# holstegelab/otter

Measured on AMD Instinct MI355X. Metric: regions/sec (otter assemble) on synthetic TR BED+BAM, 1/2/4/8 MI355X, higher is better.
Workload: dtype i16

## Files before the change

otter_amd/csrc/wfa_affine.hip:

```cpp
#include "wfa_affine_common.hpp"
#include "wfa_affine_reg.hpp"
#include "otg_chain.hpp"
#include "otg_match_queue.hpp"
#include <algorithm>
#include <cstdlib>
#include <mutex>
#include <vector>

using namespace otg_affine;

namespace {

template <int WPB>
__global__ __launch_bounds__(WPB * 64) void wfa_affine_kernel(
    const uint8_t* __restrict__ arena, const otg_align_task* __restrict__ tasks,
    const uint32_t* __restrict__ todo, const uint32_t* __restrict__ n_todo_ptr, uint32_t n_todo_imm,
    int xs, int oes, int es, int g,
    int32_t* __restrict__ scores, const uint64_t* __restrict__ cig_off, uint32_t* __restrict__ cig_len,
    uint8_t* __restrict__ cig_arena, uint64_t* __restrict__ cells,
    uint32_t* __restrict__ ticket, uint32_t* __restrict__ n_overflow, uint32_t* __restrict__ overflow_list,
    AffWs ws)
{
  constexpr int QCAP = 2048;
  __shared__ int s_lo[WPB][3][64];
// ... 734 lines not shown
  uint32_t* todo = (uint32_t*)otg_slot(ctx, SLOT_TODO, 4 * (size_t)n_tasks * sizeof(uint32_t));
  if (!cnt || !todo) return OTG_ERR_HIP;

  const size_t maxlen = ((size_t)ctx->max_seq_len + 4095) & ~(size_t)4095;
  AffWs ws = aff_ws_common(maxlen, xs, oes, es);
  ws.dbg = otg_env_set("OTG_DEBUG") ? 1 : 0; ws.visited = &cnt->visited;
  aff_ws_layout(ws, true);

  static const bool no_v3 = otg_env_set("OTG_NO_AFFINE_V3");
  static const bool no_bound = otg_env_set("OTG_NO_AFFINE_BOUND");
  static const int reg_mask_env = otg_env_int("OTG_AFFINE_REG", 31);
  static const int shape_env = otg_env_int("OTG_REG_SHAPE", 0);
  const int shape[OTG_REG_TIERS] = {(shape_env / 10000) % 10, (shape_env / 1000) % 10, (shape_env / 100) % 10, (shape_env / 10) % 10, shape_env % 10};
  const bool bounded = !no_v3 && es == 1 && xs == 2 && oes == 4 && !no_bound;
  int reg_mask = !bounded ? 0 : (maxlen <= 4096 ? (reg_mask_env & ~16) : reg_mask_env) & 31;

  constexpr int NWA = 4;
  constexpr int WPB = 4;
  AffWs wsA = ws, wsB = ws, wsC = ws, wr[OTG_REG_TIERS];
  uint32_t wavesA = 0, wavesB = 0, gridC = 2, blocks[OTG_REG_TIERS] = {0, 0, 0, 0, 0};
  const uint32_t ncu = (uint32_t)ctx->n_cu;
  {
    std::lock_guard<std::mutex> alloc_lock(otg_device_mutex(ctx->device));
    size_t free_b = 0, total_b = 0;
    HIP_TRY(ctx, hipMemGetInfo(&free_b, &total_b));
    const size_t budget = std::min<size_t>((size_t)(total_b * 0.2), (size_t)((free_b + ctx->pool[SLOT_WF_WS].cap) * 0.8));
    auto fit = [&](uint32_t& nwaves, size_t& slab) {
      while (nwaves > 1 && (ws.off_slab + slab) * (size_t)nwaves > budget) {
        if (slab > ((size_t)4 << 20)) slab /= 2; else nwaves = (nwaves + 1) / 2;
      }
    };
    auto diamond_slab = [&](size_t window) { return std::min<size_t>((size_t)(0.2 * (double)maxlen * (double)maxlen), window * window * 5 / 8) + (1 << 16); };
    wavesA = ncu * 2; size_t slabA = diamond_slab(4096);
    fit(wavesA, slabA);
    aff_ws_slab(wsA, slabA);
    wavesB = maxlen > 8192 ? ncu : ncu / 2; size_t slabB = diamond_slab(12288);
    fit(wavesB, slabB);
    aff_ws_slab(wsB, slabB);
    size_t slabC = std::min<size_t>((size_t)2 * maxlen * (size_t)(ws.nrows), budget / (gridC * WPB));
    static const size_t slab_cap_env = (size_t)otg_env_int("OTG_AFFINE_LAST_SLAB_MB", 0) << 20;
    if (slab_cap_env) slabC = std::min(slabC, slab_cap_env);
    if (slabC > ws.off_slab + 256) slabC -= ws.off_slab + 256;
    aff_ws_slab(wsC, slabC);
    const size_t need = std::max(std::max(wsA.stride * wavesA, wsB.stride * wavesB), wsC.stride * (size_t)gridC * WPB);
    uint8_t* wsp = (uint8_t*)otg_slot(ctx, SLOT_WF_WS, need);
    if (!wsp) return OTG_ERR_HIP;
    wsA.base = wsB.base = wsC.base = wsp;

    if (reg_mask) {
      HIP_TRY(ctx, hipMemGetInfo(&free_b, &total_b));
      const size_t budget_r = std::min<size_t>((size_t)(total_b * 0.25), (size_t)((free_b + ctx->pool[SLOT_REVOPS].cap) * 0.8));
      uint32_t al[OTG_REG_TIERS];
      for (int t = 0; t < OTG_REG_TIERS; ++t) {
        AffWs w = ws;
        const size_t cap = (size_t)OTG_REG_CAP[t];
        w.nrows = OTG_REG_CAP[t] + 64;
        aff_ws_layout(w, false);
        size_t slab = cap * cap * 7 / 8 + (1 << 16);
        if (t == 4) slab = std::min<size_t>(slab, (size_t)(0.2 * (double)maxlen * (double)maxlen) + (1 << 20));
        aff_ws_slab(w, slab);
        wr[t] = w;
        int apb = 1, bpc = 1;
        otg_affine_reg_geometry(t, shape[t], &apb, &bpc);
        blocks[t] = (reg_mask >> t) & 1 ? ncu * (uint32_t)bpc : 0u;
        al[t] = blocks[t] * (uint32_t)apb;
      }
      auto total = [&]() { size_t s = 256; for (int t = 0; t < OTG_REG_TIERS; ++t) s += wr[t].stride * al[t]; return s; };
      while (total() > budget_r) {
        int t = -1;
        if (blocks[4] > ncu / 4 && (wr[4].stride * al[4] >= wr[3].stride * al[3] || blocks[3] <= ncu / 2)) t = 4;
        else if (blocks[3] > ncu / 2) t = 3;
        if (t >= 0) { blocks[t] /= 2; al[t] = blocks[t]; continue; }
        for (t = OTG_REG_TIERS - 1; t >= 0 && !blocks[t]; --t) {}
        if (t < 0) break;
        blocks[t] = 0; al[t] = 0; reg_mask &= ~(1 << t);
      }
      uint8_t* wsr = reg_mask ? (uint8_t*)otg_slot(ctx, SLOT_REVOPS, total()) : nullptr;
      if (reg_mask && !wsr) {
        (void)hipGetLastError();
        reg_mask = 0;
      }
      if (ws.dbg) fprintf(stderr, "[otg] affine: register tiers keep %u / %u / %u / %u / %u alignments in flight, workspaces %.1f GB of a budget of %.1f GB, mask %d\n",
                          al[0], al[1], al[2], al[3], al[4], (double)total() / 1e9, (double)budget_r / 1e9, reg_mask);
      uint8_t* p = wsr;
      for (int t = 0; t < OTG_REG_TIERS; ++t) { wr[t].base = p; if (p) p += wr[t].stride * al[t]; }
    }
  }

  uint32_t* listA = todo;
  uint32_t* listB = todo + n_tasks;
  uint32_t* sorted = todo + 2 * (size_t)n_tasks;
  uint32_t* ovf_r = todo + 3 * (size_t)n_tasks;
  if (kernel_ms) HIP_TRY(ctx, hipEventRecord(ctx->ev0, ctx->stream));
  OtgTodo cur{d_todo, d_n_todo, n_tasks};
  if (!no_v3 && es == 1) {
    int32_t* d_bound = nullptr;
    if (bounded) {
      d_bound = (int32_t*)otg_slot(ctx, SLOT_BT_POOL, (size_t)n_tasks * sizeof(int32_t));
      if (!d_bound) return OTG_ERR_HIP;
      auto launch_bound = [&](auto kernel, uint32_t wpb, uint32_t bpc) {
        const uint32_t gridU = std::min<uint32_t>(ncu * bpc, (n_tasks + wpb - 1) / wpb);
        hipLaunchKernelGGL(kernel, dim3(gridU), dim3(wpb * 64), 0, ctx->stream, d_arena, d_tasks, d_todo, d_n_todo, n_tasks, d_bound, &cnt->bound_ticket);
      };
      if (maxlen <= 8192) launch_bound(wfa_affine_bound1_kernel<2, 4, 1030, 4>, 4, 8);
      else if (maxlen <= 12288) launch_bound(wfa_affine_bound1_kernel<2, 4, 1542, 4>, 4, 6);
      else if (maxlen <= 16384) launch_bound(wfa_affine_bound1_kernel<2, 4, 2054, 4>, 4, 4);
      else launch_bound(wfa_affine_bound1_kernel<2, 4, 4102, 2>, 2, 4);
    }
    if (d_bound && reg_mask) {
      uint32_t* hist = (uint32_t*)otg_slot(ctx, SLOT_ROWTAB, TSORT_BUCKETS * sizeof(uint32_t));
      uint32_t* seg = cnt->seg; uint32_t* n_ovf = &cnt->reg_overflow;
      if (!hist) return OTG_ERR_HIP;
      HIP_TRY(ctx, hipMemsetAsync(hist, 0, TSORT_BUCKETS * sizeof(uint32_t), ctx->stream));
      const uint32_t sg = std::min<uint32_t>((n_tasks + 2047) / 2048, ncu * 2);
      hipLaunchKernelGGL(K_tsort_hist, dim3(sg), dim3(256), 0, ctx->stream, d_todo, d_n_todo, n_tasks, d_tasks, (const int32_t*)d_bound, hist, reg_mask);
      hipLaunchKernelGGL(K_tsort_scan, dim3(1), dim3(1024), 0, ctx->stream, hist, seg);
      hipLaunchKernelGGL(K_tsort_scatter, dim3(sg), dim3(256), 0, ctx->stream, d_todo, d_n_todo, n_tasks, d_tasks, (const int32_t*)d_bound, hist, sorted, reg_mask);
      hipLaunchKernelGGL(K_seg_copy, dim3(std::min<uint32_t>((n_tasks + 255) / 256, 1024u)), dim3(256), 0, ctx->stream, (const uint32_t*)sorted,
                         (const uint32_t*)(seg + OTG_REG_TIERS), ovf_r, n_ovf);
      static const int conc_env = otg_env_int("OTG_AFFINE_CONCURRENT", -1);
      const bool concurrent = conc_env >= 0 ? conc_env != 0 : n_tasks <= 50000u;
      hipStream_t main_stream = ctx->stream;
      if (concurrent) {
        if (!ctx->ev_fork) {
          HIP_TRY(ctx, hipEventCreateWithFlags(&ctx->ev_fork, hipEventDisableTiming));
          for (int t = 0; t < OTG_REG_TIERS; ++t) {
            HIP_TRY(ctx, hipStreamCreateWithFlags(&ctx->tier_stream[t], hipStreamNonBlocking));
            HIP_TRY(ctx, hipEventCreateWithFlags(&ctx->ev_join[t], hipEventDisableTiming));
          }
        }
        HIP_TRY(ctx, hipEventRecord(ctx->ev_fork, main_stream));
      }
      int side_of[OTG_REG_TIERS] = {-2, -2, -2, -2, -2};
      int order[OTG_REG_TIERS] = {4, 3, 2, 1, 0};
      if (concurrent) {
        uint32_t hseg[OTG_REG_TIERS + 2];
        HIP_TRY(ctx, hipMemcpyAsync(hseg, seg, sizeof(hseg), hipMemcpyDeviceToHost, main_stream));
        HIP_TRY(ctx, hipStreamSynchronize(main_stream));
        static const double weight[OTG_REG_TIERS] = {1.0, 2.2, 4.0, 16.0, 64.0};
        double cost[OTG_REG_TIERS], load[3] = {0.0, 0.0, 0.0};
        for (int t = 0; t < OTG_REG_TIERS; ++t) cost[t] = blocks[t] ? weight[t] * (double)(hseg[t + 1] - hseg[t]) : 0.0;
        std::sort(order, order + OTG_REG_TIERS, [&](int a, int b) { return cost[a] > cost[b]; });
        for (int q = 0; q < OTG_REG_TIERS; ++q) {
          const int t = order[q];
          if (cost[t] <= 0.0) continue;
          int best = 0;
          for (int j = 1; j < 3; ++j) if (load[j] < load[best]) best = j;
          load[best] += cost[t];
          side_of[t] = best - 1;
        }
      } else {
        for (int t = 0; t < OTG_REG_TIERS; ++t) side_of[t] = blocks[t] ? -1 : -2;
      }
      bool side_used[2] = {false, false};
      int rc = OTG_OK; hipError_t he = hipSuccess;
      for (int q = 0; q < OTG_REG_TIERS && !rc; ++q) {
        const int t = order[q], sd = side_of[t];
        if (sd == -2) continue;
        if (sd >= 0 && !side_used[sd] && (he = hipStreamWaitEvent(ctx->tier_stream[sd], ctx->ev_fork, 0)) != hipSuccess) break;
        if (sd >= 0) { side_used[sd] = true; ctx->stream = ctx->tier_stream[sd]; }
        rc = otg_launch_affine_reg_tier(ctx, t, shape[t], blocks[t], d_arena, d_tasks, sorted, seg + t, g, d_scores, d_cig_off, d_cig_len, d_cig_arena, d_cells,
                                        &cnt->reg_ticket[t], n_ovf, ovf_r, wr[t], d_bound, &cnt->visited);
        ctx->stream = main_stream;
      }
      for (int sd = 0; sd < 2; ++sd) if (side_used[sd]) {
        if (!rc && he == hipSuccess && (he = hipEventRecord(ctx->ev_join[sd], ctx->tier_stream[sd])) == hipSuccess) he = hipStreamWaitEvent(main_stream, ctx->ev_join[sd], 0);
// ... 132 lines not shown
```

otter_amd/csrc/wfa_affine_reg.hip:

```cpp
#include "wfa_affine_common.hpp"
#include "wfa_affine_reg.hpp"
#include <cstdlib>

using namespace otg_affine;

namespace {

typedef short otg_short2 __attribute__((ext_vector_type(2)));
typedef unsigned short otg_ushort2 __attribute__((ext_vector_type(2)));

template <int I, int N, class F> __device__ __forceinline__ void static_for(F&& f)
{
  if constexpr (I < N) { f(std::integral_constant<int, I>{}); static_for<I + 1, N>(f); }
}
__device__ __forceinline__ otg_short2 as_s2(uint32_t a) { otg_short2 x; __builtin_memcpy(&x, &a, 4); return x; }
__device__ __forceinline__ otg_ushort2 as_u2(uint32_t a) { otg_ushort2 x; __builtin_memcpy(&x, &a, 4); return x; }
__device__ __forceinline__ uint32_t from_s2(otg_short2 x) { uint32_t o; __builtin_memcpy(&o, &x, 4); return o; }
__device__ __forceinline__ uint32_t from_u2(otg_ushort2 x) { uint32_t o; __builtin_memcpy(&o, &x, 4); return o; }
__device__ __forceinline__ uint32_t pk_max_i16(uint32_t a, uint32_t b) { return from_s2(__builtin_elementwise_max(as_s2(a), as_s2(b))); }
__device__ __forceinline__ uint32_t pk_add_u16(uint32_t a, uint32_t b) { return from_u2(as_u2(a) + as_u2(b)); }
__device__ __forceinline__ uint32_t pk_sub_u16(uint32_t a, uint32_t b) { return from_u2(as_u2(a) - as_u2(b)); }
__device__ __forceinline__ uint32_t pk_sub_sat_i16(uint32_t a, uint32_t b) { return from_s2(__builtin_elementwise_sub_sat(as_s2(a), as_s2(b))); }
__device__ __forceinline__ uint32_t pk_ne01_u16(uint32_t a, uint32_t b)
{
  uint32_t d, r;
  asm("v_pk_sub_u16 %0, %1, %2" : "=v"(d) : "v"(a), "v"(b));
  asm("v_pk_min_u16 %0, %1, 1 op_sel_hi:[1,0]" : "=v"(r) : "v"(d));
  return r;
}
__device__ __forceinline__ void opaque_v(int& x) { asm volatile("" : "+v"(x)); }
__device__ __forceinline__ unsigned long long mk_eq(int a, int b) { return __builtin_amdgcn_sicmp(a, b, 32); }
__device__ __forceinline__ unsigned long long mk_gt(int a, int b) { return __builtin_amdgcn_sicmp(a, b, 38); }
__device__ __forceinline__ unsigned long long mk_ule(uint32_t a, uint32_t b) { return __builtin_amdgcn_uicmp(a, b, 37); }
__device__ __forceinline__ int sel(unsigned long long m, int a, int b) { int r; asm("v_cndmask_b32_e64 %0, %1, %2, %3" : "=v"(r) : "v"(b), "v"(a), "s"(m)); return r; }
__device__ __forceinline__ int sel0(unsigned long long m, int a) { int r; asm("v_cndmask_b32_e64 %0, 0, %1, %2" : "=v"(r) : "v"(a), "s"(m)); return r; }
__device__ __forceinline__ bool lane_in(unsigned long long m, int lane) { return ((m >> lane) & 1ull) != 0ull; }
__device__ __forceinline__ void opaque_v(uint32_t& x) { asm volatile("" : "+v"(x)); }
__device__ __forceinline__ void vset(uint32_t& dst, uint32_t src) { asm("v_mov_b32 %0, %1" : "+v"(dst) : "v"(src)); }
__device__ __forceinline__ uint32_t umin3(uint32_t a, uint32_t b, uint32_t c) { const uint32_t m = a < b ? a : b; return m < c ? m : c; }
__device__ __forceinline__ uint32_t pack16(int lo, int hi) { return __builtin_amdgcn_perm((uint32_t)hi, (uint32_t)lo, 0x05040100u); }
__device__ __forceinline__ uint64_t uniform64(uint64_t x)
{
  return ((uint64_t)(uint32_t)__builtin_amdgcn_readfirstlane((int)(x >> 32)) << 32) | (uint64_t)(uint32_t)__builtin_amdgcn_readfirstlane((int)(uint32_t)x);
}

#ifndef OTG_SCHED_FENCE
#define OTG_SCHED_FENCE() __builtin_amdgcn_sched_barrier(0)
#endif

template <int NW, int S2, int SEQB, int WPEU, int QCAP = 512, int LB = 2>
__global__ __launch_bounds__(NW == 1 ? 256 : NW * 64, WPEU) void wfa_affine_reg_kernel(
    const uint8_t* __restrict__ arena, const otg_align_task* __restrict__ tasks,
    const uint32_t* __restrict__ todo, const uint32_t* __restrict__ seg, int g,
    int32_t* __restrict__ scores, const uint64_t* __restrict__ cig_off, uint32_t* __restrict__ cig_len,
    uint8_t* __restrict__ cig_arena, uint64_t* __restrict__ cells,
    uint32_t* __restrict__ ticket, uint32_t* __restrict__ n_overflow, uint32_t* __restrict__ overflow_list,
    AffWs ws, const int32_t* __restrict__ bound, unsigned long long* __restrict__ visited)
{
  constexpr int xs = 2, oes = 4, es = 1;
  constexpr int CAP = NW * S2 * 128;
  constexpr int ALN = NW == 1 ? 4 : 1;
  constexpr int WAVES = NW == 1 ? 4 : NW;
  constexpr int GS = NW * S2;
  constexpr int FAILV = -2147483647 - 1;
  constexpr int NOCAND = 0x7fffffff;
  constexpr uint32_t NN = 0x80008000u;
  constexpr uint32_t ONE2 = 0x00010001u;
  constexpr int NUL16 = -32768;
  __shared__ uint32_t s_seq[ALN][SEQB / 4];
  __shared__ uint32_t s_patch[ALN][CAP / 2];
  __shared__ uint32_t s_queue[WAVES][QCAP];
  constexpr int XROW = 2 * (GS + 2) + WAVES;
  __shared__ uint32_t s_x[2 * XROW + 64];
  __shared__ int s_misc[4];
  const int lane = threadIdx.x & 63;
  const int wv = __builtin_amdgcn_readfirstlane((int)(threadIdx.x >> 6));
  const int al = NW == 1 ? wv : 0;
  const int ww = NW == 1 ? 0 : wv;
  uint32_t* SQ = &s_seq[al][0];
  volatile lds_u32* PT = (volatile lds_u32*)&s_patch[al][0];
  volatile lds_u32* QU = (volatile lds_u32*)&s_queue[wv][0];
  volatile lds_u16* PT16 = (volatile lds_u16*)&s_patch[al][0];
  volatile lds_u32* XT = (volatile lds_u32*)&s_x[0];
  volatile __attribute__((address_space(3))) int* MISC = (volatile __attribute__((address_space(3))) int*)&s_misc[0];
  uint8_t* my = ws.base + (size_t)(blockIdx.x * ALN + al) * ws.stride;
  int64_t* rowtab = (int64_t*)(my + ws.off_rowtab);
  uint8_t* rev = my + ws.off_rev;
  uint8_t* slab = my + ws.off_slab;
  const uint32_t seg0 = seg[0], n_todo = seg[1] - seg[0];

  for (;;) {
    uint32_t tk;
    if (NW > 1) {
      if (wv == 0) MISC[0] = (int)otg_wave_atomic_add(ticket, 1u);
      __syncthreads();
      tk = (uint32_t)MISC[0];
    } else tk = otg_wave_atomic_add(ticket, 1u);
    if (tk >= n_todo) break;
    const uint32_t ti = (uint32_t)__builtin_amdgcn_readfirstlane((int)todo[seg0 + tk]);
    otg_align_task t = tasks[ti];
    t.pattern_off = uniform64(t.pattern_off); t.text_off = uniform64(t.text_off);
    t.pattern_len = (uint32_t)__builtin_amdgcn_readfirstlane((int)t.pattern_len); t.text_len = (uint32_t)__builtin_amdgcn_readfirstlane((int)t.text_len);
    t.pattern_begin_free = __builtin_amdgcn_readfirstlane(t.pattern_begin_free); t.pattern_end_free = __builtin_amdgcn_readfirstlane(t.pattern_end_free);
    t.text_begin_free = __builtin_amdgcn_readfirstlane(t.text_begin_free); t.text_end_free = __builtin_amdgcn_readfirstlane(t.text_end_free);
    t.endsfree = __builtin_amdgcn_readfirstlane(t.endsfree);
    const uint8_t* P = arena + t.pattern_off;
    const uint8_t* T = arena + t.text_off;
    const int pl = (int)t.pattern_len, tl = (int)t.text_len;
    const bool ef = t.endsfree != 0;
    const int pef = t.pattern_end_free, tef = t.text_end_free;
    const int kend = tl - pl;
    const int U = __builtin_amdgcn_readfirstlane(bound[ti]);
    const int elo = kend - (ef ? tef : 0), ehi = kend + (ef ? pef : 0);
    int lo0 = 0, hi0 = 0, kbase = 0;
    bool fail = U < 0 || U >= 0x40000000 || pl >= 32766 || tl >= 32766;
    const int offT = (pl + 15) / 16 + 3;
    if ((offT + (tl + 15) / 16 + 3) * 4 > SEQB) fail = true;
    if (!fail) {
      int need = 0;
      if (!affine_window(t, U, &kbase, &need, &lo0, &hi0) || need >= CAP) fail = true;
    }
    if (!fail) {
      for (int q = (NW == 1 ? lane : (int)threadIdx.x); q < CAP / 2; q += (NW == 1 ? 64 : NW * 64)) PT[q] = NN;
      if (NW > 1) for (int q = (int)threadIdx.x; q < 2 * XROW; q += NW * 64) XT[q] = NN;
      bool bad = false;
      auto pack = [&](const uint8_t* S, int len, int woff) {
        for (int q = (NW == 1 ? lane : (int)threadIdx.x); q < (len + 15) / 16; q += (NW == 1 ? 64 : NW * 64)) {
          uint32_t w = 0;
#pragma unroll
          for (int j = 0; j < 2; ++j) {
            const int b0 = 16 * q + 8 * j;
            const uint64_t x = b0 < len + 8 ? otg_load8(S + (b0 < len ? b0 : len)) : 0ull;
#pragma unroll
            for (int t2 = 0; t2 < 8; ++t2) {
              const uint32_t c = (uint32_t)(x >> (8 * t2)) & 0xffu;
              const uint32_t code = (c >> 1) & 3u;
              if (b0 + t2 < len && c != ((0x47544341u >> (8 * code)) & 0xffu)) bad = true;
              w |= code << (2 * (8 * j + t2));
            }
          }
          SQ[woff + q] = w;
        }
      };
      pack(P, pl, 0);
      pack(T, tl, offT);
      if ((NW == 1 ? lane : (int)threadIdx.x) < 3) { const int q3 = NW == 1 ? lane : (int)threadIdx.x; SQ[(pl + 15) / 16 + q3] = 0; SQ[offT + (tl + 15) / 16 + q3] = 0; }
      if (NW > 1) { if (threadIdx.x == 0) MISC[2] = 0; __syncthreads(); if (bad) MISC[2] = 1; __syncthreads(); fail = MISC[2] != 0; }
      else fail = __ballot(bad) != 0ull;
    }
    if (NW > 1) __syncthreads();
    __builtin_amdgcn_fence(__ATOMIC_SEQ_CST, "workgroup");
    auto ld32b = [&](int woff, int pos) -> uint64_t {
      const int w = woff + (pos >> 4);
      const uint32_t sh = (uint32_t)(pos & 15) * 2u;
      const uint32_t d0 = SQ[w], d1 = SQ[w + 1], d2 = SQ[w + 2];
      return (uint64_t)__builtin_amdgcn_alignbit(d1, d0, sh) | ((uint64_t)__builtin_amdgcn_alignbit(d2, d1, sh) << 32);
    };
    struct Ld3 { uint32_t d0, d1, d2; };
    auto ld3 = [&](int woff, int pos) -> Ld3 { const int w = woff + (pos >> 4); return Ld3{SQ[w], SQ[w + 1], SQ[w + 2]}; };
    auto cat32 = [&](const Ld3& a, int pos) -> uint64_t {
      const uint32_t sh = (uint32_t)(pos & 15) * 2u;
      return (uint64_t)__builtin_amdgcn_alignbit(a.d1, a.d0, sh) | ((uint64_t)__builtin_amdgcn_alignbit(a.d2, a.d1, sh) << 32);
    };
    auto probe_of = [&](const Ld3& p, int v, const Ld3& t, int h) -> int {
      const uint64_t x = cat32(p, v) ^ cat32(t, h);
      uint32_t flo, fhi;
      asm("v_ffbl_b32 %0, %1" : "=v"(flo) : "v"((uint32_t)x));
      asm("v_ffbl_b32 %0, %1" : "=v"(fhi) : "v"((uint32_t)(x >> 32)));
      return (int)(umin3(flo, fhi | 32u, 64u) >> 1);
    };
    auto probe32 = [&](int v, int h) -> int {
      const uint64_t x = ld32b(0, v) ^ ld32b(offT, h);
      uint32_t flo, fhi;
      asm("v_ffbl_b32 %0, %1" : "=v"(flo) : "v"((uint32_t)x));
      asm("v_ffbl_b32 %0, %1" : "=v"(fhi) : "v"((uint32_t)(x >> 32)));
      const uint32_t f = umin3(flo, fhi | 32u, 64u);
      return (int)(f >> 1);
    };
    auto match_n = [&](int v, int h, int rem, int nb) -> int {
      int m = 0;
#pragma nounroll
      for (int i = 0; i < nb; ++i) {
        if (m >= rem) break;
        const uint64_t x = ld32b(0, v + m) ^ ld32b(offT, h + m);
        if (x) { m += (int)(__builtin_ctzll(x) >> 1); break; }
        m += 32;
      }
      return m < rem ? m : rem;
    };
    auto wave_match = [&](int v, int h, int rem) -> int {
      int total = 0;
      while (total < rem) {
        const int off = total + lane * 32;
        uint64_t x = ~0ull;
        if (off < rem) x = ld32b(0, v + off) ^ ld32b(offT, h + off);
        const int m = x ? (int)(__builtin_ctzll(x) >> 1) : 32;
        const unsigned long long stop = __ballot(m < 32);
        if (stop) { const int f = (int)__builtin_ctzll(stop); total += f * 32 + __builtin_amdgcn_readlane(m, f); break; }
        total += 2048;
      }
      return total < rem ? total : rem;
    };

    uint32_t M4[2][S2], M2[2][S2];
    uint32_t WI[S2], WD[S2];
    static_for<0, S2>([&](auto ic) __attribute__((always_inline)) { constexpr int i = decltype(ic)::value;
      M4[0][i] = NN; M2[0][i] = NN; M4[1][i] = NN; M2[1][i] = NN; WI[i] = NN; WD[i] = NN;
      opaque_v(M4[0][i]); opaque_v(M2[0][i]); opaque_v(M4[1][i]); opaque_v(M2[1][i]); });
    uint32_t slab_top = 0;
    const uint32_t slab_cap = ws.slab_bytes > 0xfff00000ull ? 0xfff00000u : (uint32_t)ws.slab_bytes;
    int s_end = -1, k_end = 0;
    int r1lo = 1, r1hi = 0, r2lo = 1, r2hi = 0, r3lo = 1, r3hi = 0, r4lo = 1, r4hi = 0, idlo = 1, idhi = 0;
    uint32_t xlv = NN, xrv = NN;
    const int xe = kend - kbase;

    const int lane2_0 = 2 * lane, kb_0 = __builtin_amdgcn_readfirstlane(kbase);
    const int nul16v = NUL16;
#ifdef OTG_REG_TIMING
    unsigned long long tm_pre = 0, tm_sweep = 0, tm_drain = 0, tm_exp = 0, tm_bar = 0, tm_n = 0, tm_vis = 0, tm_last = __builtin_amdgcn_s_memtime();
#define OTG_TM(acc) { const unsigned long long now_ = __builtin_amdgcn_s_memtime(); acc += now_ - tm_last; tm_last = now_; }
#else
#define OTG_TM(acc)
#endif
    auto step = [&](auto pc, const int s) __attribute__((always_inline)) -> bool {
      constexpr int PS = decltype(pc)::value;
      const bool first = PS == 0 && s == 0;
      if (s >= ws.nrows) { fail = true; return true; }
      int lane2 = lane2_0, kb = kb_0, xes = xe;
      asm volatile("" : "+v"(lane2));
      asm volatile("" : "+s"(kb));
      asm volatile("" : "+s"(xes));
      int lo, hi;
      if (first) { lo = lo0; hi = hi0; }
      else {
        lo = 1 << 30; hi = -(1 << 30);
        if (r2hi >= r2lo) { lo = imin(lo, r2lo); hi = imax(hi, r2hi); }
        if (r4hi >= r4lo) { lo = imin(lo, r4lo - 1); hi = imax(hi, r4hi + 1); }
        if (idhi >= idlo) { lo = imin(lo, idlo - 1); hi = imax(hi, idhi + 1); }
        if (lo < -pl) lo = -pl;
        if (hi > tl) hi = tl;
        if (hi >= lo) {
          const int room = U - s;
          lo = imax(lo, elo - room); hi = imin(hi, ehi + room);
          if (room < 0 || hi < lo) { fail = true; return true; }
        }
      }
      lo = __builtin_amdgcn_readfirstlane(lo); hi = __builtin_amdgcn_readfirstlane(hi);
      r4lo = r3lo; r4hi = r3hi; r3lo = r2lo; r3hi = r2hi; r2lo = r1lo; r2hi = r1hi;
      int cand = NOCAND;
      int j0 = 1, j1 = 0;
      if (hi < lo) {
        if (PS == 0) { fail = true; return true; }
        r1lo = 1; r1hi = 0; idlo = 1; idhi = 0;
        rowtab[s] = -1;
        if (s > 2 * (oes + es * (pl + tl)) + 8) { fail = true; return true; }
      } else {
      r1lo = lo; r1hi = hi;
      const int xlo = lo - kbase, xhi = hi - kbase;
      if (xlo < 2 || xhi + 3 >= CAP) { fail = true; return true; }
      j0 = (xlo - 1) >> 7; j1 = (xhi + 1) >> 7;
      const int width = (j1 - j0 + 1) * 128;
      if (slab_top + (uint32_t)width > slab_cap) { fail = true; return true; }
      uint8_t* brow = slab + slab_top - 128 * j0;
      rowtab[s] = (int64_t)slab_top - (int64_t)(kbase + 128 * j0);
      slab_top += (uint32_t)width;
      int qn = 0;
      auto drain = [&]() {
        int pass = 0;
        while (qn > 0) {
          if (qn <= 4 && pass > 0) {
            for (int e = 0; e < qn; ++e) {
              const uint32_t ent = (uint32_t)__builtin_amdgcn_readfirstlane((int)QU[e]);
              const int x = (int)(ent & 0xffffu), h = (int)(ent >> 16), kk = kbase + x, v = h - kk;
              const int m = wave_match(v, h, imin(pl - v, tl - h));
              const int hf = h + m, vf = v + m;
              PT16[x] = (uint16_t)hf;
              if (ef ? ((hf >= tl && pl - vf <= pef) || (vf >= pl && tl - hf <= tef)) : (x == xe && hf >= tl)) cand = imin(cand, kk);
            }
            qn = 0;
            break;
          }
          int wq = 0;
          for (int q0 = 0; q0 < qn; q0 += 64) {
            const bool act = q0 + lane < qn;
            int x = 0, kk = 0, h = 0, v = 0;
            bool more = false, fin = false;
            if (act) {
              const uint32_t ent = QU[q0 + lane];
              x = (int)(ent & 0xffffu); h = (int)(ent >> 16); kk = kbase + x; v = h - kk;
              const int rem = imin(pl - v, tl - h);
              int m, full;
              if (pass == 0) { m = match_n(v, h, rem, 2); full = 64; }
              else { m = match_n(v, h, rem, 8); full = 256; }
              v += m; h += m;
              more = (m == full) && v < pl && h < tl;
              if (!more) {
                PT16[x] = (uint16_t)h;
                fin = ef ? ((h >= tl && pl - v <= pef) || (v >= pl && tl - h <= tef)) : (x == xe && h >= tl);
              }
            }
            const unsigned long long fm = __ballot(fin);
            if (fm) {
              int kc = fin ? kk : NOCAND;
              kc = -otg_wave_max_i32(-kc);
              cand = imin(cand, kc);
            }
            const unsigned long long mm = __ballot(more);
            if (more) {
              const int rank = (int)__builtin_amdgcn_mbcnt_hi((uint32_t)(mm >> 32), __builtin_amdgcn_mbcnt_lo((uint32_t)mm, 0u));
              QU[wq + rank] = (uint32_t)x | ((uint32_t)h << 16);
            }
            wq += __builtin_popcountll(mm);
          }
          qn = wq; ++pass;
        }
      };
      constexpr int QFULL = 2 * QCAP;
      auto push2 = [&](bool moreE, bool moreO, unsigned long long mE, unsigned long long mO, int xE, int hE, int hO) {
        if (mE | mO) {
          if (qn + 128 > QCAP) { qn = QFULL; return; }
          const int nE = __builtin_popcountll(mE);
          if (moreE) {
            const int rank = (int)__builtin_amdgcn_mbcnt_hi((uint32_t)(mE >> 32), __builtin_amdgcn_mbcnt_lo((uint32_t)mE, 0u));
            QU[qn + rank] = (uint32_t)xE | ((uint32_t)hE << 16);
          }
          if (moreO) {
            const int rank = (int)__builtin_amdgcn_mbcnt_hi((uint32_t)(mO >> 32), __builtin_amdgcn_mbcnt_lo((uint32_t)mO, 0u));
            QU[qn + nE + rank] = (uint32_t)(xE + 1) | ((uint32_t)hO << 16);
          }
          qn += nE + __builtin_popcountll(mO);
        }
      };
      auto fin_ef = [&](int h, int v) -> bool { return h >= 0 && ((h >= tl && pl - v <= pef) || (v >= pl && tl - h <= tef)); };

      OTG_TM(tm_pre);
      if (first) {
        static_for<0, S2>([&](auto ic) __attribute__((always_inline)) { constexpr int i = decltype(ic)::value;
          const int gi = NW == 1 ? i : i * NW + ww;
          if (gi < j0 || gi > j1) return;
          const int xE = 128 * gi + lane2, kE = kb + xE, kO = kE + 1;
          const int hE = kE > 0 ? kE : 0, vE = hE - kE, hO = kO > 0 ? kO : 0, vO = hO - kO;
          const bool validE = kE >= lo && kE <= hi && hE <= tl && vE <= pl, validO = kO >= lo && kO <= hi && hO <= tl && vO <= pl;
          M2[PS][i] = pack16(validE ? hE - 1 : NUL16, validO ? hO - 1 : NUL16);
// ... 32 lines not shown
          uint32_t bw = neM + (neM & neD);
          bw = ((fI >> 13) & 0x00040004u) | bw;
          bw = ((fD >> 12) & 0x00080008u) | bw;
          bw ^= 0x000C000Cu;
          const uint16_t b2 = (uint16_t)__builtin_amdgcn_perm(bw, bw, 0x0c0c0200u);
          const int xE = 128 * gi + lane2, kE = kb + xE;
          __builtin_memcpy(brow + 128 * gi + (uint32_t)lane2, &b2, 2);
          WI[i] = Inew; WD[i] = Dnew;
          int hE = (int)(int16_t)(Mx & 0xffffu), hO = (int)Mx >> 16;
          const int vE = hE - kE, vO = hO - kE - 1;
          const unsigned long long vmE = mk_ule((uint32_t)hE, (uint32_t)tl) & mk_ule((uint32_t)vE, (uint32_t)pl);
          const unsigned long long vmO = mk_ule((uint32_t)hO, (uint32_t)tl) & mk_ule((uint32_t)vO, (uint32_t)pl);
          const int rvE = pl - vE, rhE = tl - hE, rvO = pl - vO, rhO = tl - hO;
          int mE, mO;
          if constexpr (LB == 2) {
            const Ld3 pE = ld3(0, vE), tE = ld3(offT, hE), pO = ld3(0, vO), tO = ld3(offT, hO);
            OTG_SCHED_FENCE();
            mE = imin(probe_of(pE, vE, tE, hE), imin(rvE, rhE));
            mO = imin(probe_of(pO, vO, tO, hO), imin(rvO, rhO));
            OTG_SCHED_FENCE();
          } else if constexpr (LB == 1) {
            OTG_SCHED_FENCE();
            { const Ld3 pE = ld3(0, vE), tE = ld3(offT, hE); OTG_SCHED_FENCE(); mE = imin(probe_of(pE, vE, tE, hE), imin(rvE, rhE)); }
            OTG_SCHED_FENCE();
            { const Ld3 pO = ld3(0, vO), tO = ld3(offT, hO); OTG_SCHED_FENCE(); mO = imin(probe_of(pO, vO, tO, hO), imin(rvO, rhO)); }
            OTG_SCHED_FENCE();
          } else {
            OTG_SCHED_FENCE();
            mE = imin(probe32(vE, hE), imin(rvE, rhE));
            OTG_SCHED_FENCE();
            mO = imin(probe32(vO, hO), imin(rvO, rhO));
            OTG_SCHED_FENCE();
          }
          hE += mE; hO += mO;
          unsigned long long mmE = vmE & mk_eq(mE, 32) & mk_gt(rvE, 32) & mk_gt(rhE, 32), mmO = vmO & mk_eq(mO, 32) & mk_gt(rvO, 32) & mk_gt(rhO, 32);
          if ((mmE | mmO) != 0ull) {
            const unsigned long long selO = mmO & ~mmE;
            const int h2 = sel(selO, hO, hE);
            const int v2 = h2 - sel(selO, kE + 1, kE);
            const int rv2 = pl - v2, rh2 = tl - h2;
            int m2nd;
            if constexpr (LB > 0) { const Ld3 p2 = ld3(0, v2), t2 = ld3(offT, h2); OTG_SCHED_FENCE(); m2nd = imin(probe_of(p2, v2, t2, h2), imin(rv2, rh2)); }
            else m2nd = imin(probe32(v2, h2), imin(rv2, rh2));
            const unsigned long long m2m = mk_eq(m2nd, 32) & mk_gt(rv2, 32) & mk_gt(rh2, 32);
            hO += sel0(selO, m2nd); hE += sel0(mmE, m2nd);
            mmO &= mmE | m2m; mmE &= m2m;
          }
          M4[PS][i] = m2;
          M2[PS][i] = pack16(sel(vmE, hE, nul16v), sel(vmO, hO, nul16v));
          if (ef) {
            const int hp = pl + kE;
            if ((mk_eq(hE, tl) | mk_eq(hE, hp) | mk_eq(hO, tl) | mk_eq(hO, hp + 1)) != 0ull) {
              const bool fE = lane_in(vmE & ~mmE, lane) && fin_ef(hE, hE - kE), fO = lane_in(vmO & ~mmO, lane) && fin_ef(hO, hO - kE - 1);
              const unsigned long long fm = __ballot(fE || fO);
              if (fm) { int kc = fE ? kE : (fO ? kE + 1 : NOCAND); kc = -otg_wave_max_i32(-kc); cand = imin(cand, kc); }
            }
          } else if ((xes >> 7) == gi) {
            const bool odd = (xes & 1) != 0;
            const int hx = __builtin_amdgcn_readlane(sel(odd ? (vmO & ~mmO) : (vmE & ~mmE), odd ? hO : hE, -1), (xes & 127) >> 1);
            if (hx >= tl) cand = kend;
          }
          if ((mmE | mmO) != 0ull) push2(lane_in(mmE, lane), lane_in(mmO, lane), mmE, mmO, xE, hE, hO);
        });
      }
      if (first) static_for<0, S2>([&](auto ic) __attribute__((always_inline)) { constexpr int i = decltype(ic)::value; M4[PS][i] = NN; opaque_v(M4[PS][i]); });
      OTG_TM(tm_sweep);
#ifdef OTG_REG_TIMING
      tm_n += 1; tm_vis += (unsigned long long)(NW == 1 ? (j1 - j0 + 1) : ((j1 - ww + NW) / NW - (j0 - ww + NW - 1) / NW));
#endif
      if (qn >= QFULL) cand = FAILV;
      else if (qn > 0) {
        drain();
        static_for<0, S2>([&](auto ic) __attribute__((always_inline)) { constexpr int i = decltype(ic)::value;
          const int gi = NW == 1 ? i : i * NW + ww;
          if (gi < j0 || gi > j1) return;
          const int pi = 64 * gi + (lane2 >> 1);
          const uint32_t pw = PT[pi];
          if (__ballot(pw != NN)) {
            M2[PS][i] = pk_max_i16(M2[PS][i], pw);
            PT[pi] = NN;
          }
        });
      }
      idlo = first ? 1 : lo; idhi = first ? 0 : hi;
      OTG_TM(tm_drain);
      }
      cand = __builtin_amdgcn_readfirstlane(cand);
      if (NW > 1) {
        constexpr int np = (1 - PS) * XROW;
        if (lane == 0 || lane == 63) {
          volatile lds_u32* dst = XT + np + (lane == 63 ? 0 : GS + 2) + ww + 1;
          static_for<0, S2>([&](auto ic) __attribute__((always_inline)) { constexpr int i = decltype(ic)::value;
            dst[i * NW] = pk_max_i16(M4[1 - PS][i], lane == 63 ? WI[i] : WD[i]); });
          if (lane == 0) XT[np + 2 * (GS + 2) + ww] = (uint32_t)cand;
        }
        OTG_TM(tm_exp);
        __syncthreads();
        xlv = XT[np + lane];
        xrv = XT[np + GS + 4 + lane];
        const int cv = (int)XT[np + 2 * (GS + 2) + (lane & (WAVES - 1))];
        int gc = NOCAND;
#pragma unroll
        for (int w2 = 0; w2 < NW; ++w2) { const int c2 = __builtin_amdgcn_readlane(cv, w2); gc = c2 < gc ? c2 : gc; }
        cand = __builtin_amdgcn_readfirstlane(gc);
        OTG_TM(tm_bar);
      }
      if (cand == FAILV) fail = true;
      else if (cand != NOCAND) { s_end = s; k_end = cand; }
      return fail || s_end >= 0;
    };
    for (int s = 0; !fail; s += 2) {
      if (step(std::integral_constant<int, 0>{}, s)) break;
      if (step(std::integral_constant<int, 1>{}, s + 1)) break;
    }

#ifdef OTG_REG_TIMING
    if (visited && lane == 0) {
      atomicAdd(visited + 2, tm_pre); atomicAdd(visited + 3, tm_sweep); atomicAdd(visited + 4, tm_drain); atomicAdd(visited + 5, tm_exp);
      atomicAdd(visited + 6, tm_bar); atomicAdd(visited + 7, tm_n); atomicAdd(visited + 8, tm_vis);
    }
#endif
    if (NW > 1 && wv != 0) continue;
    if (fail || s_end < 0) {
      const uint32_t q = otg_wave_atomic_add(n_overflow, 1u);
      overflow_list[q] = ti;
      continue;
    }
    __builtin_amdgcn_fence(__ATOMIC_SEQ_CST, "agent");
    if (!backtrace_unpack<true>(P, pl, T, tl, s_end, k_end, xs, oes, es, rowtab, slab, rev, ws.rev_cap, cig_arena + cig_off[ti], lane, &scores[ti], &cig_len[ti], g,
                                (volatile lds_u32*)&s_queue[wv][0], EqPacked{(volatile lds_u32*)&s_seq[al][0], offT})) continue;
    if (cells) cells[ti] = affine_cells(t, xs, oes, s_end);
    if (visited && lane == 0) atomicAdd(visited, (unsigned long long)slab_top);
  }
}

}

void otg_affine_reg_geometry(int tier, int shape, int* aln_per_block, int* blocks_per_cu)
{
  int a = 4, b = 4;
  switch (tier * 10 + shape) {
    case 0: a = 4; b = 4; break;
    case 1: a = 1; b = 10; break;
    case 10: a = 4; b = 3; break;
    case 11: a = 4; b = 4; break;
    case 12: a = 1; b = 8; break;
    case 20: a = 1; b = 8; break;
    case 21: a = 4; b = 3; break;
    case 22: a = 4; b = 2; break;
    case 30: a = 1; b = 4; break;
    case 31: a = 1; b = 3; break;
    case 40: a = 1; b = 2; break;

    default: break;
  }
  *aln_per_block = a; *blocks_per_cu = b;
}

int otg_launch_affine_reg_tier(otg_ctx* ctx, int tier, int shape, uint32_t blocks, const uint8_t* d_arena, const otg_align_task* d_tasks,
                               const uint32_t* d_sorted, const uint32_t* d_seg, int g, int32_t* d_scores, const uint64_t* d_cig_off,
                               uint32_t* d_cig_len, uint8_t* d_cig_arena, uint64_t* d_cells, uint32_t* ticket, uint32_t* n_overflow,
                               uint32_t* overflow_list, const AffWs& ws, const int32_t* d_bound, unsigned long long* visited)
{
#define OTG_REG_LAUNCH(NWV, S2V, SEQV, WPEUV, ...)                                                                                              \
  hipLaunchKernelGGL((wfa_affine_reg_kernel<NWV, S2V, SEQV, WPEUV, ##__VA_ARGS__>), dim3(blocks), dim3(NWV == 1 ? 256 : NWV * 64), 0, ctx->stream, d_arena, \
                     d_tasks, d_sorted, d_seg, g, d_scores, d_cig_off, d_cig_len, d_cig_arena, d_cells, ticket, n_overflow, overflow_list, ws, d_bound, visited)
  switch (tier * 10 + shape) {
    case 0: OTG_REG_LAUNCH(1, 8, 4096, 4); break;
    case 30: OTG_REG_LAUNCH(4, 8, 8192, 4); break;
#ifndef OTG_REG_PROBE
    case 1: OTG_REG_LAUNCH(2, 4, 4096, 5, 256); break;
    case 10: OTG_REG_LAUNCH(1, 12, 4608, 3); break;
    case 11: OTG_REG_LAUNCH(1, 12, 4608, 4, 512, 0); break;
    case 12: OTG_REG_LAUNCH(2, 6, 4608, 4); break;
    case 20: OTG_REG_LAUNCH(2, 8, 6144, 4); break;
    case 21: OTG_REG_LAUNCH(1, 16, 6144, 3, 512, 1); break;
    case 22: OTG_REG_LAUNCH(1, 16, 6144, 2); break;
    case 31: OTG_REG_LAUNCH(8, 4, 8192, 6, 256); break;
    case 40: OTG_REG_LAUNCH(8, 8, 12288, 4); break;

#endif
    default: return otg_fail(ctx, OTG_ERR_ARG, "no register tier %d shape %d", tier, shape);
  }
#undef OTG_REG_LAUNCH
  HIP_TRY(ctx, hipGetLastError());
  return OTG_OK;
}
```

otter_amd/csrc/wfa_affine_reg.hpp:

```cpp
#pragma once
#include "wfa_affine_common.hpp"

constexpr int OTG_REG_CAP[OTG_REG_TIERS] = {1024, 1536, 2048, 4096, 8192};
constexpr int OTG_REG_SEQB[OTG_REG_TIERS] = {4096, 4608, 6144, 8192, 12288};
void otg_affine_reg_geometry(int tier, int shape, int* aln_per_block, int* blocks_per_cu);

int otg_launch_affine_reg_tier(otg_ctx* ctx, int tier, int shape, uint32_t blocks, const uint8_t* d_arena, const otg_align_task* d_tasks,
                               const uint32_t* d_sorted, const uint32_t* d_seg, int g, int32_t* d_scores, const uint64_t* d_cig_off,
                               uint32_t* d_cig_len, uint8_t* d_cig_arena, uint64_t* d_cells, uint32_t* ticket, uint32_t* n_overflow,
                               uint32_t* overflow_list, const otg_affine::AffWs& ws, const int32_t* d_bound, unsigned long long* visited);
```

Measured before the change: 18800.

## Compute affine diagonal range in closed form and trim register-tier LDS

Replaces the per-score rolling range bookkeeping (r1..r4, id ranges) in the register-tier WFA kernel with a closed-form diagonal band computed from the score. Score 0 and the empty score 1 are peeled out of the loop so `first` becomes a compile-time flag. The cross-wave LDS buffers are now allocated only for multi-wave shapes, and blocks-per-CU is raised for several tiers. A debug occupancy query is also added. The closed-form band may be wider than the tracked one, which means more diagonals are computed per score. The empty-row handling and its early-fail check are removed, which risks changing behaviour on edge cases.

```diff
diff --git a/otter_amd/csrc/affine_score_range.hpp b/otter_amd/csrc/affine_score_range.hpp
--- /dev/null
+++ b/otter_amd/csrc/affine_score_range.hpp
@@ -0,0 +1,32 @@
+#pragma once
+
+#if defined(__HIPCC__)
+#define OTG_RANGE_HD __host__ __device__ __forceinline__
+#else
+#define OTG_RANGE_HD inline
+#endif
+
+namespace otg_affine {
+
+enum { RANGE_FAIL = -1, RANGE_EMPTY = 0, RANGE_OK = 1 };
+
+OTG_RANGE_HD int affine_score_range(int s, int lo0, int hi0, int pl, int tl, int U, int elo, int ehi, int* lo, int* hi)
+{
+  if (s == 0) { *lo = lo0; *hi = hi0; return hi0 >= lo0 ? RANGE_OK : RANGE_FAIL; }
+  if (s == 1) { *lo = 1; *hi = 0; return RANGE_EMPTY; }
+  const int g = s - 2;
+  int l = lo0 - g, h = hi0 + g;
+  if (l < -pl) l = -pl;
+  if (h > tl) h = tl;
+  if (h >= l) {
+    const int room = U - s;
+    const int dl = elo - room, dh = ehi + room;
+    if (l < dl) l = dl;
+    if (h > dh) h = dh;
+    if (room < 0 || h < l) return RANGE_FAIL;
+  }
+  *lo = l; *hi = h;
+  return h >= l ? RANGE_OK : RANGE_EMPTY;
+}
+
+}
diff --git a/otter_amd/csrc/wfa_affine.hip b/otter_amd/csrc/wfa_affine.hip
--- a/otter_amd/csrc/wfa_affine.hip
+++ b/otter_amd/csrc/wfa_affine.hip
@@ -840,6 +840,18 @@
       }
       if (ws.dbg) fprintf(stderr, "[otg] affine: register tiers keep %u / %u / %u / %u / %u alignments in flight, workspaces %.1f GB of a budget of %.1f GB, mask %d\n",
                           al[0], al[1], al[2], al[3], al[4], (double)total() / 1e9, (double)budget_r / 1e9, reg_mask);
+      if (ws.dbg) for (int t = 0; t < OTG_REG_TIERS; ++t) {
+        if (!((reg_mask >> t) & 1)) continue;
+        int apb = 1, bpc = 1, occ = 0, lds = 0, vg = 0;
+        otg_affine_reg_geometry(t, shape[t], &apb, &bpc);
+        if (otg_affine_reg_occupancy(ctx, t, shape[t], &occ, &lds, &vg) != OTG_OK) {
+          (void)hipGetLastError();
+          fprintf(stderr, "[otg] affine: register tier %d shape %d: %d blocks per CU launched, the runtime's figure n/a\n", t, shape[t], bpc);
+          continue;
+        }
+        fprintf(stderr, "[otg] affine: register tier %d shape %d: %d blocks per CU launched, the runtime co-schedules %d (LDS %d bytes per block, %d vector registers)\n",
+                t, shape[t], bpc, occ, lds, vg);
+      }
       uint8_t* p = wsr;
       for (int t = 0; t < OTG_REG_TIERS; ++t) { wr[t].base = p; if (p) p += wr[t].stride * al[t]; }
     }
diff --git a/otter_amd/csrc/wfa_affine_reg.hip b/otter_amd/csrc/wfa_affine_reg.hip
--- a/otter_amd/csrc/wfa_affine_reg.hip
+++ b/otter_amd/csrc/wfa_affine_reg.hip
@@ -1,4 +1,5 @@
 #include "wfa_affine_common.hpp"
+#include "affine_score_range.hpp"
 #include "wfa_affine_reg.hpp"
 #include <cstdlib>
 
@@ -42,6 +43,12 @@
 __device__ __forceinline__ uint64_t uniform64(uint64_t x)
 {
   return ((uint64_t)(uint32_t)__builtin_amdgcn_readfirstlane((int)(x >> 32)) << 32) | (uint64_t)(uint32_t)__builtin_amdgcn_readfirstlane((int)(uint32_t)x);
+}
+
+template <int ID, int N> __device__ __forceinline__ uint32_t* lds_words()
+{
+  if constexpr (N > 0) { __shared__ uint32_t w[N]; return &w[0]; }
+  else return nullptr;
 }
 
 #ifndef OTG_SCHED_FENCE
@@ -71,8 +78,8 @@
   __shared__ uint32_t s_patch[ALN][CAP / 2];
   __shared__ uint32_t s_queue[WAVES][QCAP];
   constexpr int XROW = 2 * (GS + 2) + WAVES;
-  __shared__ uint32_t s_x[2 * XROW + 64];
-  __shared__ int s_misc[4];
+  uint32_t* s_x = lds_words<0, (NW > 1 ? 2 * XROW + 64 : 0)>();
+  uint32_t* s_misc = lds_words<1, (NW > 1 ? 4 : 0)>();
   const int lane = threadIdx.x & 63;
   const int wv = __builtin_amdgcn_readfirstlane((int)(threadIdx.x >> 6));
   const int al = NW == 1 ? wv : 0;
@@ -210,7 +217,6 @@
     uint32_t slab_top = 0;
     const uint32_t slab_cap = ws.slab_bytes > 0xfff00000ull ? 0xfff00000u : (uint32_t)ws.slab_bytes;
     int s_end = -1, k_end = 0;
-    int r1lo = 1, r1hi = 0, r2lo = 1, r2hi = 0, r3lo = 1, r3hi = 0, r4lo = 1, r4hi = 0, idlo = 1, idhi = 0;
     uint32_t xlv = NN, xrv = NN;
     const int xe = kend - kbase;
 
@@ -222,43 +228,21 @@
 #else
 #define OTG_TM(acc)
 #endif
-    auto step = [&](auto pc, const int s) __attribute__((always_inline)) -> bool {
+    auto step = [&](auto pc, auto fc, const int s) __attribute__((always_inline)) -> bool {
       constexpr int PS = decltype(pc)::value;
-      const bool first = PS == 0 && s == 0;
+      constexpr bool first = decltype(fc)::value;
       if (s >= ws.nrows) { fail = true; return true; }
       int lane2 = lane2_0, kb = kb_0, xes = xe;
       asm volatile("" : "+v"(lane2));
       asm volatile("" : "+s"(kb));
       asm volatile("" : "+s"(xes));
       int lo, hi;
-      if (first) { lo = lo0; hi = hi0; }
-      else {
-        lo = 1 << 30; hi = -(1 << 30);
-        if (r2hi >= r2lo) { lo = imin(lo, r2lo); hi = imax(hi, r2hi); }
-        if (r4hi >= r4lo) { lo = imin(lo, r4lo - 1); hi = imax(hi, r4hi + 1); }
-        if (idhi >= idlo) { lo = imin(lo, idlo - 1); hi = imax(hi, idhi + 1); }
-        if (lo < -pl) lo = -pl;
-        if (hi > tl) hi = tl;
-        if (hi >= lo) {
-          const int room = U - s;
-          lo = imax(lo, elo - room); hi = imin(hi, ehi + room);
-          if (room < 0 || hi < lo) { fail = true; return true; }
-        }
-      }
+      if (affine_score_range(s, lo0, hi0, pl, tl, U, elo, ehi, &lo, &hi) != RANGE_OK) { fail = true; return true; }
       lo = __builtin_amdgcn_readfirstlane(lo); hi = __builtin_amdgcn_readfirstlane(hi);
-      r4lo = r3lo; r4hi = r3hi; r3lo = r2lo; r3hi = r2hi; r2lo = r1lo; r2hi = r1hi;
       int cand = NOCAND;
-      int j0 = 1, j1 = 0;
-      if (hi < lo) {
-        if (PS == 0) { fail = true; return true; }
-        r1lo = 1; r1hi = 0; idlo = 1; idhi = 0;
-        rowtab[s] = -1;
-        if (s > 2 * (oes + es * (pl + tl)) + 8) { fail = true; return true; }
-      } else {
-      r1lo = lo; r1hi = hi;
       const int xlo = lo - kbase, xhi = hi - kbase;
       if (xlo < 2 || xhi + 3 >= CAP) { fail = true; return true; }
-      j0 = (xlo - 1) >> 7; j1 = (xhi + 1) >> 7;
+      const int j0 = (xlo - 1) >> 7, j1 = (xhi + 1) >> 7;
       const int width = (j1 - j0 + 1) * 128;
       if (slab_top + (uint32_t)width > slab_cap) { fail = true; return true; }
       uint8_t* brow = slab + slab_top - 128 * j0;
@@ -457,16 +441,15 @@
           }
         });
       }
-      idlo = first ? 1 : lo; idhi = first ? 0 : hi;
       OTG_TM(tm_drain);
-      }
       cand = __builtin_amdgcn_readfirstlane(cand);
       if (NW > 1) {
-        constexpr int np = (1 - PS) * XROW;
+        constexpr int NP = first ? PS : 1 - PS;
+        constexpr int np = first ? 0 : (1 - PS) * XROW;
         if (lane == 0 || lane == 63) {
           volatile lds_u32* dst = XT + np + (lane == 63 ? 0 : GS + 2) + ww + 1;
           static_for<0, S2>([&](auto ic) __attribute__((always_inline)) { constexpr int i = decltype(ic)::value;
-            dst[i * NW] = pk_max_i16(M4[1 - PS][i], lane == 63 ? WI[i] : WD[i]); });
+            dst[i * NW] = pk_max_i16(M4[NP][i], lane == 63 ? WI[i] : WD[i]); });
           if (lane == 0) XT[np + 2 * (GS + 2) + ww] = (uint32_t)cand;
         }
         OTG_TM(tm_exp);
@@ -484,9 +467,15 @@
       else if (cand != NOCAND) { s_end = s; k_end = cand; }
       return fail || s_end >= 0;
     };
-    for (int s = 0; !fail; s += 2) {
-      if (step(std::integral_constant<int, 0>{}, s)) break;
-      if (step(std::integral_constant<int, 1>{}, s + 1)) break;
+    if (!fail && !step(std::integral_constant<int, 0>{}, std::true_type{}, 0)) {
+      if (1 >= ws.nrows) fail = true;
+      else {
+        rowtab[1] = -1;
+        for (int s = 2;; s += 2) {
+          if (step(std::integral_constant<int, 0>{}, std::false_type{}, s)) break;
+          if (step(std::integral_constant<int, 1>{}, std::false_type{}, s + 1)) break;
+        }
+      }
     }
 
 #ifdef OTG_REG_TIMING
@@ -517,19 +506,55 @@
   switch (tier * 10 + shape) {
     case 0: a = 4; b = 4; break;
     case 1: a = 1; b = 10; break;
-    case 10: a = 4; b = 3; break;
+    case 10: a = 4; b = 4; break;
     case 11: a = 4; b = 4; break;
     case 12: a = 1; b = 8; break;
-    case 20: a = 1; b = 8; break;
+    case 20: a = 1; b = 10; break;
     case 21: a = 4; b = 3; break;
     case 22: a = 4; b = 2; break;
-    case 30: a = 1; b = 4; break;
+    case 30: a = 1; b = 5; break;
     case 31: a = 1; b = 3; break;
     case 40: a = 1; b = 2; break;
 
     default: break;
   }
   *aln_per_block = a; *blocks_per_cu = b;
+}
+
+#ifndef OTG_REG_PROBE
+#define OTG_REG_SHAPES(X)    \
+  X(0, 1, 8, 4096, 4)        \
+  X(30, 4, 8, 8192, 4)       \
+  X(1, 2, 4, 4096, 5, 256)   \
+  X(10, 1, 12, 4608, 3)      \
+  X(11, 1, 12, 4608, 4, 512, 0) \
+  X(12, 2, 6, 4608, 4)       \
+  X(20, 2, 8, 6144, 4)       \
+  X(21, 1, 16, 6144, 3, 512, 1) \
+  X(22, 1, 16, 6144, 2)      \
+  X(31, 8, 4, 8192, 6, 256)  \
+  X(40, 8, 8, 12288, 4)
+#else
+#define OTG_REG_SHAPES(X) X(0, 1, 8, 4096, 4) X(30, 4, 8, 8192, 4)
+#endif
+
+int otg_affine_reg_occupancy(otg_ctx* ctx, int tier, int shape, int* blocks_per_cu, int* lds_bytes, int* vgprs)
+{
+  hipFuncAttributes at{};
+  int nb = 0;
+#define OTG_REG_QUERY(CASE, NWV, S2V, SEQV, WPEUV, ...)                                                                                             \
+  case CASE: {                                                                                                                                       \
+    auto kern = wfa_affine_reg_kernel<NWV, S2V, SEQV, WPEUV, ##__VA_ARGS__>;                                                                         \
+    HIP_TRY(ctx, hipOccupancyMaxActiveBlocksPerMultiprocessor(&nb, kern, NWV == 1 ? 256 : NWV * 64, 0));                                             \
+    HIP_TRY(ctx, hipFuncGetAttributes(&at, reinterpret_cast<const void*>(kern)));                                                                    \
+  } break;
+  switch (tier * 10 + shape) {
+    OTG_REG_SHAPES(OTG_REG_QUERY)
+    default: return otg_fail(ctx, OTG_ERR_ARG, "no register tier %d shape %d", tier, shape);
+  }
+#undef OTG_REG_QUERY
+  *blocks_per_cu = nb; *lds_bytes = (int)at.sharedSizeBytes; *vgprs = at.numRegs;
+  return OTG_OK;
 }
 
 int otg_launch_affine_reg_tier(otg_ctx* ctx, int tier, int shape, uint32_t blocks, const uint8_t* d_arena, const otg_align_task* d_tasks,
@@ -537,24 +562,13 @@
                                uint32_t* d_cig_len, uint8_t* d_cig_arena, uint64_t* d_cells, uint32_t* ticket, uint32_t* n_overflow,
                                uint32_t* overflow_list, const AffWs& ws, const int32_t* d_bound, unsigned long long* visited)
 {
-#define OTG_REG_LAUNCH(NWV, S2V, SEQV, WPEUV, ...)                                                                                              \
-  hipLaunchKernelGGL((wfa_affine_reg_kernel<NWV, S2V, SEQV, WPEUV, ##__VA_ARGS__>), dim3(blocks), dim3(NWV == 1 ? 256 : NWV * 64), 0, ctx->stream, d_arena, \
-                     d_tasks, d_sorted, d_seg, g, d_scores, d_cig_off, d_cig_len, d_cig_arena, d_cells, ticket, n_overflow, overflow_list, ws, d_bound, visited)
+#define OTG_REG_LAUNCH(CASE, NWV, S2V, SEQV, WPEUV, ...)                                                                                        \
+  case CASE:                                                                                                                                     \
+    hipLaunchKernelGGL((wfa_affine_reg_kernel<NWV, S2V, SEQV, WPEUV, ##__VA_ARGS__>), dim3(blocks), dim3(NWV == 1 ? 256 : NWV * 64), 0, ctx->stream, d_arena, \
+                       d_tasks, d_sorted, d_seg, g, d_scores, d_cig_off, d_cig_len, d_cig_arena, d_cells, ticket, n_overflow, overflow_list, ws, d_bound, visited); \
+    break;
   switch (tier * 10 + shape) {
-    case 0: OTG_REG_LAUNCH(1, 8, 4096, 4); break;
-    case 30: OTG_REG_LAUNCH(4, 8, 8192, 4); break;
-#ifndef OTG_REG_PROBE
-    case 1: OTG_REG_LAUNCH(2, 4, 4096, 5, 256); break;
-    case 10: OTG_REG_LAUNCH(1, 12, 4608, 3); break;
-    case 11: OTG_REG_LAUNCH(1, 12, 4608, 4, 512, 0); break;
-    case 12: OTG_REG_LAUNCH(2, 6, 4608, 4); break;
-    case 20: OTG_REG_LAUNCH(2, 8, 6144, 4); break;
-    case 21: OTG_REG_LAUNCH(1, 16, 6144, 3, 512, 1); break;
-    case 22: OTG_REG_LAUNCH(1, 16, 6144, 2); break;
-    case 31: OTG_REG_LAUNCH(8, 4, 8192, 6, 256); break;
-    case 40: OTG_REG_LAUNCH(8, 8, 12288, 4); break;
-
-#endif
+    OTG_REG_SHAPES(OTG_REG_LAUNCH)
     default: return otg_fail(ctx, OTG_ERR_ARG, "no register tier %d shape %d", tier, shape);
   }
 #undef OTG_REG_LAUNCH
diff --git a/otter_amd/csrc/wfa_affine_reg.hpp b/otter_amd/csrc/wfa_affine_reg.hpp
--- a/otter_amd/csrc/wfa_affine_reg.hpp
+++ b/otter_amd/csrc/wfa_affine_reg.hpp
@@ -4,6 +4,7 @@
 constexpr int OTG_REG_CAP[OTG_REG_TIERS] = {1024, 1536, 2048, 4096, 8192};
 constexpr int OTG_REG_SEQB[OTG_REG_TIERS] = {4096, 4608, 6144, 8192, 12288};
 void otg_affine_reg_geometry(int tier, int shape, int* aln_per_block, int* blocks_per_cu);
+int otg_affine_reg_occupancy(otg_ctx* ctx, int tier, int shape, int* blocks_per_cu, int* lds_bytes, int* vgprs);
 
 int otg_launch_affine_reg_tier(otg_ctx* ctx, int tier, int shape, uint32_t blocks, const uint8_t* d_arena, const otg_align_task* d_tasks,
                                const uint32_t* d_sorted, const uint32_t* d_seg, int g, int32_t* d_scores, const uint64_t* d_cig_off,
```

After: 20410, median of 6. 1.09x the previous value.
